# superxslam/SuperOdom

Measured on AMD Instinct MI355X. Metric: icp_registrations_per_sec, higher is better.
Workload: dtype f64

## Files before the change

### include/so_icp.h

```cpp
#ifndef SO_ICP_H
#define SO_ICP_H

#include <stddef.h>
#include <stdint.h>

#ifdef __cplusplus
extern "C" {
#endif

#define SO_ICP_ABI_VERSION 4

#define SO_ICP_MAP_W 21
#define SO_ICP_MAP_H 21
#define SO_ICP_MAP_D 11
#define SO_ICP_MAP_NUM 4851
#define SO_ICP_MAX_OUTER 16

#define SO_ICP_OK 0
#define SO_ICP_NOT_ENOUGH_MAP_FEATURES 1
#define SO_ICP_MAP_SEEDED 2
#define SO_ICP_STAGE_DECLINED 3
#define SO_ICP_E_INVALID (-1)
#define SO_ICP_E_HIP (-2)
#define SO_ICP_E_NOMEM (-3)
// ... 70 lines not shown
#define SO_ICP_FLAG_RETRIED 0x2u
#define SO_ICP_FLAG_HOST_MAP 0x4u
#define SO_ICP_FLAG_SORT_BINNING 0x8u
#define SO_ICP_FLAG_SHARDED 0x10u
#define SO_ICP_FLAG_STAGED_SCAN 0x20u
#define SO_ICP_FLAG_COPY_READBACK 0x40u
#define SO_ICP_FLAG_QUERY_SPLIT 0x80u
#define SO_ICP_FLAG_BINNED_AHEAD 0x100u
#define SO_ICP_FLAG_QUERY_WAVES 0x200u

#define SO_ICP_FLAG_CHAINED 0x400u
#define SO_ICP_FLAG_POSE_PRIOR 0x800u

typedef struct {
  double knn_ms_total;   int64_t knn_launches;   int64_t knn_queries;   int64_t knn_map_points;
  double eval_ms_total;  int64_t eval_launches;  int64_t eval_points;
  double prep_ms_total;  int64_t prep_launches;
  double host_ms_total;  int64_t registrations;
  int64_t knn_group_passes, knn_fallback_lanes, knn_candidates_scanned;
  double stage_wait_ms_total;  int64_t staged_direct, staged_copied, stage_declined;
  int64_t knn_packed_rows, knn_packed_rows_too_many_runs, knn_packed_rows_tile_full, knn_packed_kept;
  int64_t knn_pack_registrations, knn_pack_holds;
  int64_t seq_chained, seq_chain_breaks;
} so_icp_timing;

void so_icp_default_config(so_icp_config *cfg);
so_icp_ctx *so_icp_create(const so_icp_config *cfg);
void so_icp_destroy(so_icp_ctx *ctx);
const char *so_icp_last_error(const so_icp_ctx *ctx);
int so_icp_abi_version(void);
int so_icp_device_available(void);
int so_icp_device_count(void);

int so_icp_set_resolution(so_icp_ctx *ctx, float line_res, float plane_res);
int so_icp_set_max_surface_features(so_icp_ctx *ctx, int max_surface_features);
int so_icp_set_max_iterations(so_icp_ctx *ctx, int max_iterations);
int so_icp_set_cloud_intensity(so_icp_ctx *ctx, int offset_bytes);

int so_icp_map_set_origin(so_icp_ctx *ctx, const double t_w_cur[3], int origin_out[3]);
int so_icp_map_shift(so_icp_ctx *ctx, const double t_w_cur[3], int pos_in_map[3]);
int so_icp_map_add_surf(so_icp_ctx *ctx, const float *xyz, size_t n, size_t stride_bytes);
int so_icp_map_count_5x5(so_icp_ctx *ctx, const int pos[3], int *n_edge, int *n_surf);
int so_icp_map_export(so_icp_ctx *ctx, float *xyz, size_t cap_points, size_t *n_out, int only_5x5, const int pos[3]);
int so_icp_map_export_records(so_icp_ctx *ctx, void *out, size_t stride_bytes, size_t cap_points, size_t *n_out, int only_5x5, const int pos[3]);
int so_icp_map_size(so_icp_ctx *ctx, size_t *n_points, size_t *n_points_this_rank);
int so_icp_map_clear(so_icp_ctx *ctx);
// ... 302 lines not shown
```

### superodom_amd/binding.py

```python
import ctypes as C
import math
import os

import numpy as np

HERE = os.path.dirname(os.path.abspath(__file__))
LIB_PATH = os.path.join(HERE, "lib", "libsoicp.so")
N_REJECT, N_OBS, MAX_OUTER, UID_BYTES, PEER_HANDLE_BYTES = 7, 9, 16, 128, 80

OK, NOT_ENOUGH_MAP_FEATURES, MAP_SEEDED = 0, 1, 2
SHARD_MAP, SHARD_QUERIES = 0, 1


class Config(C.Structure):
    _fields_ = [("abi_version", C.c_int32), ("device_id", C.c_int32), ("rank", C.c_int32), ("world_size", C.c_int32),
                ("max_iterations", C.c_int32), ("lm_max_iterations", C.c_int32), ("max_surface_features", C.c_int32),
                ("k", C.c_int32), ("tukey_variant", C.c_int32), ("time_kernels", C.c_int32),
                ("line_res", C.c_float), ("plane_res", C.c_float), ("yaw_ratio", C.c_double),
                ("velocity_failure_threshold", C.c_double), ("shard_mode", C.c_int32), ("solve_workgroups", C.c_int32)]


class IterStats(C.Structure):
    _fields_ = [("translation_norm", C.c_double), ("rotation_norm", C.c_double), ("num_surf_from_scan", C.c_int32),
                ("num_corner_from_scan", C.c_int32), ("lm_iterations", C.c_int32), ("num_successful_steps", C.c_int32),
# ... 105 lines not shown
def untimed_layout(fields, point_step, row_step, n_scans, filter_point_size, min_range, is_bigendian=False):
    off = {}
    for name in ("x", "y", "z", "intensity"):
        for fname, foff, fdt, fcount in fields:
            if fname == name and fdt == FLOAT32 and (fcount == 1 or fcount == 0):
                off[name] = int(foff)
                break
    L = UntimedLayout()
    L.is_bigendian, L.point_step, L.row_step = int(bool(is_bigendian)), int(point_step), int(row_step)
    L.off_x, L.off_y, L.off_z, L.off_intensity = off.get("x", -1), off.get("y", -1), off.get("z", -1), off.get("intensity", -1)
    L.n_scans, L.filter_point_size, L.min_range = int(n_scans), int(filter_point_size), float(min_range)
    return L


class Timing(C.Structure):
    _fields_ = [("knn_ms_total", C.c_double), ("knn_launches", C.c_int64), ("knn_queries", C.c_int64), ("knn_map_points", C.c_int64),
                ("eval_ms_total", C.c_double), ("eval_launches", C.c_int64), ("eval_points", C.c_int64),
                ("prep_ms_total", C.c_double), ("prep_launches", C.c_int64),
                ("host_ms_total", C.c_double), ("registrations", C.c_int64),
                ("knn_group_passes", C.c_int64), ("knn_fallback_lanes", C.c_int64), ("knn_candidates_scanned", C.c_int64),
                ("stage_wait_ms_total", C.c_double), ("staged_direct", C.c_int64), ("staged_copied", C.c_int64), ("stage_declined", C.c_int64),
                ("knn_packed_rows", C.c_int64), ("knn_packed_rows_too_many_runs", C.c_int64), ("knn_packed_rows_tile_full", C.c_int64),
                ("knn_packed_kept", C.c_int64), ("knn_pack_registrations", C.c_int64), ("knn_pack_holds", C.c_int64),
                ("seq_chained", C.c_int64), ("seq_chain_breaks", C.c_int64)]


class Sums(C.Structure):
    _fields_ = [("cost", C.c_double), ("count", C.c_double), ("Jtr", C.c_double * 6), ("JtJ", C.c_double * 21), ("hist", C.c_double * 16)]


class LmState(C.Structure):
    _fields_ = [("opaque", C.c_double * 96)]


class LmScriptEntry(C.Structure):
    _fields_ = [("sums", Sums), ("new_solve", C.c_int32), ("reserved", C.c_int32)]


class LmScriptStep(C.Structure):
    _fields_ = [("more", C.c_int32), ("reserved", C.c_int32), ("pose", C.c_double * 7), ("hand", (C.c_uint32 * 4) * 8), ("state", LmState)]


class LmScriptResult(C.Structure):
    _fields_ = [("state", LmState), ("T", C.c_double * 7), ("eval_pose", C.c_double * 7), ("T_final", C.c_double * 7),
                ("JtJ", C.c_double * 36), ("Jtr", C.c_double * 6),
                ("lm_more", C.c_int32), ("outer_iter", C.c_int32), ("n_iterations", C.c_int32), ("reg_done", C.c_int32),
                ("done_count", C.c_uint32), ("reserved", C.c_uint32), ("iterations", IterStats * 16)]
# ... 984 lines not shown
```

### superodom_amd/csrc/ctx.h

```cpp
#pragma once
#include <hip/hip_runtime_api.h>
#include <rccl/rccl.h>

#include <atomic>
#include <chrono>
#include <condition_variable>
#include <cstdint>
#include <cstring>
#include <memory>
#include <mutex>
#include <string>
#include <thread>
#include <vector>

#include "../../include/so_icp.h"
#include "device_map.h"
#include "kernels.h"
#include "local_map.h"
#include "lm_solver.h"
#include "reg_plan.h"
#include "so_math.h"

namespace soicp::host {

// ... 252 lines not shown
  bool prebin = true;
  BinHashTable pbin;
  StageSlot* stage_in_use = nullptr;
  unsigned long long stage_seq = 0, stage_consumed_seq = 0;
  bool stage_quit = false, stage_started = false;
  std::atomic<int> stage_pending{0};
  std::atomic<bool> stage_parked{false};
  std::atomic<bool> stage_timed{false};
  std::thread stage_thread; std::mutex stage_mu; std::condition_variable stage_cv;
  struct HostRange { const char* p; size_t bytes; bool owned; };
  std::vector<HostRange> host_ranges;
  hipStream_t seq_stream = nullptr;
  StageSlot seq_slot[kStageSlots];
  BinHashTable sbin;
  int seq_depth = 2; uint32_t done_count_seen = 0;
  struct SeqNext { const void* next_scan = nullptr; size_t next_n = 0; double delta[7] = {0, 0, 0, 0, 0, 0, 1}; bool announced = false;
                   const void* scan = nullptr; size_t n = 0;
                   bool staged = false; int slot = 0; bool binned = false, needs_event = false; const float* d_scan = nullptr; } seq_next;
  bool seq_chain = true;
  bool query_waves = true;
  bool knn_pack = true;
  bool knn_list_fits = false;
  uint32_t packed_leftover_seen = 0;
  int knn_pack_hold = 0;
  static constexpr int kBatchRoundsTracked = 16;
  float batch_survivors[kBatchRoundsTracked] = {};
  bool batch_chain = true;
  hipStream_t copy_stream = nullptr;
  bool retried = false;
  unsigned long long peer_timeout_ticks = 100000000ull;
  bool scan_staged = false;
  bool query_split = false;
  DevBuf d_sub;

  ~so_icp_ctx();
};

#define HIP_TRY(ctx, expr)                                                                         \
  do {                                                                                             \
    hipError_t e__ = (expr);                                                                       \
    if (e__ != hipSuccess) {                                                                       \
      (ctx)->err = std::string(#expr) + ": " + hipGetErrorString(e__);                             \
      return SO_ICP_E_HIP;                                                                         \
    }                                                                                              \
  } while (0)

// ... 106 lines not shown
```

### superodom_amd/csrc/icp_context.cpp

```cpp
#include <hip/hip_runtime_api.h>

#include <algorithm>
#include <atomic>
#include <chrono>
#include <cmath>
#include <cstdlib>
#include <cstring>
#include <new>
#include <string>
#include <thread>
#include <vector>

#include "ctx.h"

static_assert(sizeof(so_icp_sums) == sizeof(LmSums), "so_icp_sums must mirror LmSums");
static_assert(sizeof(LmState) <= sizeof(so_icp_lm_state), "so_icp_lm_state too small");
static_assert(sizeof(LmSums) == 45 * sizeof(double), "LmSums is 45 doubles");

namespace soicp::host {

thread_local std::string g_create_error;

hipEvent_t next_event(so_icp_ctx* c) {
  if (c->ev_used == c->ev_pool.size()) {
// ... 149 lines not shown
  for (unsigned spin = 1;; ++spin) {
    if (*seq == want) break;
    if ((spin & 0x3FFu) != 0) continue;
    const auto now = std::chrono::steady_clock::now();
    if (now < next_check) continue;
    next_check = now + std::chrono::milliseconds(1);
    if (hipStreamQuery(s) != hipErrorNotReady) {
      (void)hipGetLastError();
      if (*seq == want) break;
      const hipError_t e = hipStreamSynchronize(s);
      if (e != hipSuccess) { c->err = std::string("hipStreamSynchronize(s): ") + hipGetErrorString(e); return Report::kHipError; }
      if (*seq == want) break;
      return Report::kDrained;
    }
  }
  std::atomic_thread_fence(std::memory_order_acquire);
  return Report::kReported;
}
void note_registration_done(so_icp_ctx* c, DevState* mirror, const MatchParams& mp, size_t n, bool sets_list_fits, bool sets_done_count) {
  const DevState& H = *(c->h_state = mirror);
  if (mp.pack_light) c->timing.knn_pack_registrations++;
  const uint32_t packed_left = H.packed_leftover >= c->packed_leftover_seen ? H.packed_leftover - c->packed_leftover_seen : H.packed_leftover;
  c->packed_leftover_seen = H.packed_leftover;
  if (mp.pack_light && (double)packed_left > 0.03 * (double)n * (double)std::max(H.n_iterations, 1)) { c->knn_pack_hold = 32; c->timing.knn_pack_holds++; }
  if (sets_list_fits) c->knn_list_fits = work_list_fits(H.bin_packed, (unsigned long long)kKnnBlocks * 4ull);
  if (sets_done_count) c->done_count_seen = H.done_count;
}

static void uncertainty_from_hist(const int32_t* H, double u[6]) {
  const double tt = (double)H[6] + H[7] + H[8];
  const double tr = (double)H[0] + H[1] + H[2] + H[3] + H[4] + H[5];
  if (tt == 0 || tr == 0) { for (int i = 0; i < 6; ++i) u[i] = 0; return; }
  u[0] = std::fmin(H[6] / tt * 3, 1.0); u[1] = std::fmin(H[7] / tt * 3, 1.0); u[2] = std::fmin(H[8] / tt * 3, 1.0);
  u[3] = std::fmin((H[0] + H[1]) / tr * 3, 1.0); u[4] = std::fmin((H[2] + H[3]) / tr * 3, 1.0); u[5] = std::fmin((H[4] + H[5]) / tr * 3, 1.0);
}

static void yaw_correction(double T[7], const double last[7], double yaw_ratio) {
  double tn, rn;
  relative_motion(last, T, tn, rn);
  const float translation_norm = (float)tn;
  const double x = T[3], y = T[4], z = T[5], w = T[6];
  const double d = x * x + y * y + z * z + w * w, s = 2.0 / d;
  const double xs = x * s, ys = y * s, zs = z * s, wx = w * xs, wy = w * ys, wz = w * zs;
  const double xx = x * xs, xy = x * ys, xz = x * zs, yy = y * ys, yz = y * zs, zz = z * zs;
  const double m00 = 1.0 - (yy + zz), m01 = xy - wz, m02 = xz + wy, m10 = xy + wz, m20 = xz - wy, m21 = yz + wx, m22 = 1.0 - (xx + yy);
  double roll, pitch, yaw;
// ... 936 lines not shown
```

### superodom_amd/csrc/kernels.h

```cpp
#pragma once
#include <hip/hip_runtime_api.h>

#include <cstddef>
#include <cstdint>

#include "lm_endgame.h"
#include "lm_solver.h"
#include "pose_prior.h"
#include "so_math.h"

#ifndef SO_ENDGAME_IMAGE
#define SO_ENDGAME_IMAGE 1
#endif
#ifndef SO_PUBLISH_FENCED
#define SO_PUBLISH_FENCED 0
#endif
#ifndef SO_PTOL_AT_PROPOSAL
#define SO_PTOL_AT_PROPOSAL 1
#endif

namespace soicp {

struct DevMapView {
  const float4* pts;
// ... 47 lines not shown
  unsigned long long timeout_ticks;
};
constexpr int kPeerMaxWorld = 8, kPeerChunks = 48;
constexpr size_t kPeerInboxBytes = (size_t)(2 * kPeerMaxWorld * kPeerChunks + kPeerMaxWorld) * 16;

struct CorrBuffers {
  double4* nd;
  double* coeff;
  uint8_t* status;
};

struct DevIterStats {
  double translation_norm, rotation_norm;
  int32_t num_surf, lm_iterations, num_successful, termination;
  double initial_cost, final_cost;
  int32_t reject_hist[7], obs_hist[9];
  double pose_after[7];
};
struct DevState {
  double pose_in[7];
  int32_t max_outer, lm_max, pad0, pad1;
  int32_t outer_iter, reg_done, lm_more, n_iterations;
  uint32_t packed_leftover;
  uint32_t pad2[3];
  unsigned long long bin_packed;
  double T[7];
  double eval_pose[7];
  LmState S;
  double JtJ[36], Jtr[6];
  DevIterStats iters[16];
  double T_final[7];
  double T_chain[7];
  uint32_t done_count, pad3;
  unsigned long long peer_seq;
  unsigned long long dbg[16];
  unsigned long long seq;
};
static_assert(sizeof(DevState) % 8 == 0, "DevState is copied in 8-byte words");

constexpr int kHistReplicas = 16;
constexpr int kHistStride = 32;
constexpr int kKnnBlocks = 1024;
#ifndef SO_SOLVE_BLOCKS
#define SO_SOLVE_BLOCKS 256
#endif
constexpr int kEvalBlocks = SO_SOLVE_BLOCKS;
constexpr int kFitBlocksMax = SO_SOLVE_BLOCKS;
// ... 86 lines not shown
```

### superodom_amd/csrc/kernels.hip

```cpp
#include <hip/hip_runtime.h>
#include <hip/hip_ext.h>

#include <cstddef>
#include <cstdlib>
#include <cstring>
#include <type_traits>

#ifdef SO_LM_STAMPS
#define SO_LM_STAMP(dbg, i) do { if (dbg) (dbg)[i] = wall_clock64(); } while (0)
#endif
#include "device_idioms.h"
#include "kernels.h"
#include "plane_factor.h"
#include "plane_fit.h"
#include "pose_prior.h"

namespace soicp {

#define SO_MATCH_SUCCESS 0
#define SO_MATCH_NOT_ENOUGH 1
#define SO_MATCH_TOO_FAR 2
#define SO_MATCH_BAD_PCA 3
#define SO_MATCH_INVALID 4
#define SO_MATCH_MSE 5
// ... 407 lines not shown
__device__ __forceinline__ float block_cover_distance(int bx0, int bx1, int by0, int by1, int bz0, int bz1, int nc, float cell,
                                                      float ux, float uy, float uz) {
  float cv = 1e15f;
  if (bx0 > 0) cv = fminf(cv, ux - (float)bx0 * cell);
  if (bx1 < nc - 1) cv = fminf(cv, (float)(bx1 + 1) * cell - ux);
  if (by0 > 0) cv = fminf(cv, uy - (float)by0 * cell);
  if (by1 < nc - 1) cv = fminf(cv, (float)(by1 + 1) * cell - uy);
  if (bz0 > 0) cv = fminf(cv, uz - (float)bz0 * cell);
  if (bz1 < nc - 1) cv = fminf(cv, (float)(bz1 + 1) * cell - uz);
  return fmaxf(cv - 1e-4f, 0.f);
}
__device__ __forceinline__ void survivors_to_canon(const Net8& net, const uint32_t* tile_canon, uint32_t n_valid, uint32_t tile_cap,
                                                   uint32_t (&canon)[8]) {
  const int32_t ks[8] = {net.a0, net.a1, net.a2, net.a3, net.a4, net.a5, net.a6, net.a7};
#pragma unroll
  for (int t = 0; t < 8; ++t) {
    const uint32_t jl = (uint32_t)ks[t] & kKeyIdxMask;
    canon[t] = (ks[t] == kKeyEmpty || jl >= n_valid) ? 0xFFFFFFFFu : tile_canon[jl < tile_cap ? jl : 0u];
  }
}
#ifndef SO_KNN_PACK
#define SO_KNN_PACK 1
#endif
constexpr uint32_t kPartTile = kTileCand / 4;

template <bool PROF, bool BATCH, int BEGIN = 0>
__global__ __launch_bounds__(256, 4) void knn_plane_kernel(const float4* __restrict__ binned ,
                                                        const uint32_t* __restrict__ chunk_start,
                                                        const DevState* __restrict__ st,
                                                        const float4* __restrict__ mpts,
                                                        const uint32_t* __restrict__ mcell_start, DevMapView map,
                                                        MatchParams mp, CorrBuffers corr, uint32_t* __restrict__ nbr5,
                                                        int32_t* __restrict__ hist, BatchView bv) {
  __shared__ int32_t lh[24];
  __shared__ __attribute__((aligned(16))) float tiles[4][4][kTileCand + 16];
  __shared__ uint32_t tcanon[4][kTileCand + 16];
  __shared__ uint32_t rowtab[4][2][72];
  unsigned long long t_entry = 0;
  if (PROF) t_entry = wall_clock64();
  if (SO_ENTRY_WARM) st = after_loaded(st, kernarg_lines<decltype(&knn_plane_kernel<PROF, BATCH, BEGIN>)>());
  if (BATCH) {
    const size_t h = bv.active[blockIdx.y];
    st += h; binned += h * bv.bs; chunk_start += h * bv.bs;
    corr.status += h * bv.bs; nbr5 += h * 5 * bv.bs; hist += h * (kHistReplicas * kHistStride);
  }
  uint32_t* const leftover_ctr = (BATCH && mp.packed_leftover)
      ? reinterpret_cast<uint32_t*>(reinterpret_cast<char*>(mp.packed_leftover) + (size_t)bv.active[blockIdx.y] * sizeof(DevState)) : mp.packed_leftover;
  constexpr bool begin = BEGIN != 0 && !BATCH;
// ... 54 lines not shown
  if (stamp) { ts[0] = wall_clock64(); if (!n_mine) t_item0 = ts[0]; }
  uint32_t j = 0;
  bool valid_q = false;
  bool split = false, split4 = false;
  const uint32_t part = (uint32_t)lane >> 4, lane16 = (uint32_t)lane & 15u;
  if constexpr (packed) {
    const uint32_t li = chunk * 4u + part;
    const uint32_t desc = li < n_light ? chunk_start[mp.chunk_cap - 1u - li] : 0u;
    const uint32_t start = desc & 0x03FFFFFFu, count = li < n_light ? (desc >> 26) + 1u : 0u;
    j = start + lane16;
    valid_q = (lane16 < count) && (j < n_kept);
  } else {
    const uint32_t entry = pack ? chunk - n_packed
                         : (chunk < n_light1 ? mp.chunk_cap - 1u - chunk
                            : (chunk < n_light1 + n_normal ? chunk - n_light1 : mp.chunk_cap - 1u - (chunk - n_normal)));
    const uint32_t desc = __builtin_amdgcn_readfirstlane(chunk_start[entry]);
    const uint32_t start = desc & 0x03FFFFFFu, count = (desc >> 26) + 1u;
    split = count <= 32u && !(abl & 1024);
    split4 = count <= 16u && split && !(abl & 2048);
    const int ql = split4 ? (lane & 15) : (split ? (lane & 31) : lane);
    j = start + (uint32_t)ql;
    valid_q = (ql < (int)count) && (j < n_kept);
  }
  const uint32_t hoff = split4 ? (uint32_t)(lane >> 4) << 2 : (split ? (uint32_t)(lane >> 5) << 2 : 0u);
  const uint32_t sstep = split4 ? 16u : 8u;
  double pw[3] = {0, 0, 0};
  float qx = 0, qy = 0, qz = 0;
  float ux = 0, uy = 0, uz = 0;
  int wcube0 = 0, wcube1 = 0, wcube2 = 0;
  CellRef c;
  c.slot = -1; c.cx = c.cy = c.cz = 0;
  uint32_t oi = 0;
  if (valid_q) {
    const float4 rec = binned[j];
    oi = __float_as_uint(rec.w);
    quat_rotate<double>(pose.q, (double)rec.x, (double)rec.y, (double)rec.z, pw[0], pw[1], pw[2]);
    pw[0] += pose.t[0]; pw[1] += pose.t[1]; pw[2] += pose.t[2];
    qx = (float)pw[0]; qy = (float)pw[1]; qz = (float)pw[2];
    int w[3] = {0, 0, 0};
    c = locate(map, qx, qy, qz, w);
    if (c.slot >= 0) {
      ux = (float)((double)qx - (w[0] * 50.0 - 25.0)); uy = (float)((double)qy - (w[1] * 50.0 - 25.0)); uz = (float)((double)qz - (w[2] * 50.0 - 25.0));
      wcube0 = w[0]; wcube1 = w[1]; wcube2 = w[2];
    }
  }
  const uint32_t ckey = (valid_q && c.slot >= 0) ? (((uint32_t)c.slot << 18) | ((uint32_t)c.cz << 12) | ((uint32_t)c.cy << 6) | (uint32_t)c.cx)
                                                 : 0xFFFFFFFFu;
  Top5 top;
  top.init();
  bool resolved = (ckey == 0xFFFFFFFFu);
  bool too_far_certain = false, need_exact = false;
  int n_groups = 0;
  uint32_t n_scanned = 0, n_left_stat = 0;
  if (stamp) { ts[1] = wall_clock64(); acc[0] += ts[1] - ts[0]; }
  auto certify = [qx, qy, qz, mpts, &mp](int pass, const uint32_t (&gs)[8], int32_t k6, int32_t k8, float cov2, Top5& top) -> int {
    unsigned long long e[5];
#pragma unroll
    for (int t = 0; t < 5; ++t) {
      e[t] = ~0ull;
      if (gs[t] != 0xFFFFFFFFu) {
        const float4 p = mpts[gs[t]];
        e[t] = ((unsigned long long)__float_as_uint(l2_d2(qx, qy, qz, p.x, p.y, p.z)) << 32) | gs[t];
      }
    }
    top.set5(e[0], e[1], e[2], e[3], e[4]);
    const double cov = (double)cov2 * (1.0 - 1e-6);
    double R2 = cov;
    if (k6 != kKeyEmpty) R2 = fmin(R2, (double)__uint_as_float((uint32_t)k6 & ~kKeyIdxMask) * (1.0 - 1e-6) - (double)kApproxAbsErr);
    bool have5 = top.b4 != ~0ull;
    double d5 = (double)__uint_as_float((uint32_t)(top.b4 >> 32));
    bool exact = have5 && d5 < R2;
    bool far = !exact && R2 > (double)mp.sq_max_dist_f;
    if (__ballot(!exact && !far && gs[5] != 0xFFFFFFFFu)) {
      if (!exact && !far) {
#pragma unroll
        for (int t = 5; t < 8; ++t) {
// ... 23 lines not shown
    const bool mine = pend && myslot == gslot;
    const float r_cover = ppass == 0 ? r_near : r_gate;
    const int lo_x = max(0, (int)floorf((ux - r_cover) * inv_cellf)), hi_x = min(nc - 1, (int)floorf((ux + r_cover) * inv_cellf));
    const int lo_y = max(0, (int)floorf((uy - r_cover) * inv_cellf)), hi_y = min(nc - 1, (int)floorf((uy + r_cover) * inv_cellf));
    const int lo_z = max(0, (int)floorf((uz - r_cover) * inv_cellf)), hi_z = min(nc - 1, (int)floorf((uz + r_cover) * inv_cellf));
    const int bx0 = row_min_i32(mine ? lo_x : 0x7FFFFFFF), bx1 = row_max_i32(mine ? hi_x : -1);
    const int by0 = row_min_i32(mine ? lo_y : 0x7FFFFFFF), by1 = row_max_i32(mine ? hi_y : -1);
    const int bz0 = row_min_i32(mine ? lo_z : 0x7FFFFFFF), bz1 = row_max_i32(mine ? hi_z : -1);
    const int nyr = by1 - by0 + 1, nrows = nyr * (bz1 - bz0 + 1);
    bool part_ok = gslot != 0x7FFFFFFF && nrows >= 1 && nrows <= 16;
    float cv = block_cover_distance(bx0, bx1, by0, by1, bz0, bz1, nc, cell, ux, uy, uz);
    if (ppass == 1) cv = 1e15f;
    const float cov2p = fminf(cv * cv, r_cover * r_cover);
    uint32_t vb = 0, vl = 0;
    if (part_ok && (int)lane16 < nrows) {
      const int zq = (int)(((float)lane16 + 0.5f) * __builtin_amdgcn_rcpf((float)nyr));
      const int z = bz0 + zq, y = by0 + ((int)lane16 - zq * nyr);
      const uint32_t* row = mcell_start + (size_t)gslot * map.ncell1 + ((size_t)z * nc + y) * nc;
      vb = row[bx0]; vl = row[bx1 + 1] - vb;
    }
    const uint32_t inc = row_inclusive_scan_u32(vl);
    const uint32_t total = (uint32_t)row_max_i32((int)inc);
    part_ok = part_ok && total <= 1024u;
    uint32_t* prowoff = rowoff + part * 17u;
    uint32_t* prowbeg = rowbeg + part * 16u;
    wave_lds_fence();
    prowoff[lane16] = ((int)lane16 < nrows) ? inc - vl : total; prowbeg[lane16] = vb;
    if (lane16 == 0) prowoff[16] = total;
    const int gz = (bz0 + bz1) >> 1, gy = (by0 + by1) >> 1, gx = (bx0 + bx1) >> 1;
    const int w0r = row_max_i32(mine ? wcube0 : -0x7FFFFFFF), w1r = row_max_i32(mine ? wcube1 : -0x7FFFFFFF), w2r = row_max_i32(mine ? wcube2 : -0x7FFFFFFF);
    const double rox = (w0r * 50.0 - 25.0) + ((double)gx + 0.5) * (double)cell;
    const double roy = (w1r * 50.0 - 25.0) + ((double)gy + 0.5) * (double)cell;
    const double roz = (w2r * 50.0 - 25.0) + ((double)gz + 0.5) * (double)cell;
    const float lqx = (float)((double)qx - rox), lqy = (float)((double)qy - roy), lqz = (float)((double)qz - roz);
    const float m2qx = -2.f * lqx, m2qy = -2.f * lqy, m2qz = -2.f * lqz;
    const float qq = __builtin_fmaf(lqz, lqz, __builtin_fmaf(lqy, lqy, lqx * lqx));
    const float pinf = __int_as_float(0x7F800000);
    const float bl0 = row_min_f32(mine ? lqx : pinf), bl1 = row_min_f32(mine ? lqy : pinf), bl2 = row_min_f32(mine ? lqz : pinf);
    const float bh0 = -row_min_f32(mine ? -lqx : pinf), bh1 = -row_min_f32(mine ? -lqy : pinf), bh2 = -row_min_f32(mine ? -lqz : pinf);
    const float dk = r_cover + 2e-4f, dk2 = dk * dk;
    const uint32_t tbase = part * kPartTile;
    const uint32_t tot_eff = part_ok ? total : 0u;
    const uint32_t tmax = max_over_rows(tot_eff);
    wave_lds_fence();
    if (PROF) n_scanned += tmax;
    uint32_t w = 0;
// ... 143 lines not shown
      if (lane == L) {
        top.b0 = m5[0]; top.b1 = m5[1]; top.b2 = m5[2]; top.b3 = m5[3]; top.b4 = m5[4];
        too_far_certain = false; resolved = true;
      }
  };
  if constexpr (packed) {
    unsigned long long left = __ballot(valid_q && c.slot >= 0 && !resolved);
    if (left) __builtin_amdgcn_s_setprio(3);
    if (left && lane == 0 && mp.packed_leftover) atomicAdd(leftover_ctr, (uint32_t)__popcll(left));
    if (PROF) n_left_stat = (uint32_t)__popcll(left);
    while (left) {
      const int L = __ffsll((long long)left) - 1;
      left &= left - 1ull;
      coop_exact_scan(L);
    }
  }
  if constexpr (!packed)
  for (int pass = first_pass; pass < 2; ++pass) {
  bool pending = !resolved && !need_exact;
  unsigned long long todo = __ballot(pending);
  if (abl & 2) todo = 0;
  if (!todo) continue;
  if (pass == 1 && first_pass == 0) __builtin_amdgcn_s_setprio(3);
  if (stamp && pass == 1) ++n_pass2;
  const float r_cover = pass == 0 ? r_near : r_gate;
  const int lo_x = max(0, (int)floorf((ux - r_cover) * inv_cellf)), hi_x = min(nc - 1, (int)floorf((ux + r_cover) * inv_cellf));
  const int lo_y = max(0, (int)floorf((uy - r_cover) * inv_cellf)), hi_y = min(nc - 1, (int)floorf((uy + r_cover) * inv_cellf));
  const int lo_z = max(0, (int)floorf((uz - r_cover) * inv_cellf)), hi_z = min(nc - 1, (int)floorf((uz + r_cover) * inv_cellf));
  uint32_t g0 = 0xFFFFFFFFu, g1 = g0, g2 = g0, g3 = g0, g4 = g0, g5 = g0, g6 = g0, g7 = g0;
  int32_t k6 = kKeyEmpty, k8 = kKeyEmpty;
  float cov2 = 0.f;
  bool scanned = false;
  while (todo) {
    const int leader = __ffsll((long long)todo) - 1;
    const uint32_t k = __builtin_amdgcn_readlane(ckey, leader);
    const int gslot = (int)(k >> 18);
    bool mine = pending && ((int)(ckey >> 18) == gslot);
    int bx0, bx1, by0, by1, bz0, bz1;
    uint32_t total = 0;
    uint32_t vb = 0, vl = 0;
    int nrows = 0, nyr = 0;
    const int lcx = (int)(k & 63u), lcy = (int)((k >> 6) & 63u), lcz = (int)((k >> 12) & 63u);
    for (int attempt = 0; attempt < 3; ++attempt) {
      if (attempt == 1)
        mine = mine && abs(c.cx - lcx) <= 1 && abs(c.cy - lcy) <= 1 && abs(c.cz - lcz) <= 1;
      if (attempt == 2) mine = mine && (ckey == k);
      bx0 = __builtin_amdgcn_readlane(lo_x, leader); bx1 = __builtin_amdgcn_readlane(hi_x, leader);
// ... 23 lines not shown
        if (lane == 0) rowoff[32] = total;
      }
      if (total <= kGroupMaxCand) break;
    }
    pending = pending && !mine;
    todo = __ballot(pending);
    ++n_groups;
    if (total > kGroupMaxCand) {
      need_exact = need_exact || mine;
      continue;
    }
    n_scanned += total;
    if (n_scanned > 256u) __builtin_amdgcn_s_setprio(3);
    else if (n_scanned > 128u) __builtin_amdgcn_s_setprio(2);
    if (stamp) { ts[2] = wall_clock64(); acc[1] += ts[2] - ts[1]; }
    const int gz = (bz0 + bz1) >> 1, gy = (by0 + by1) >> 1, gx = (bx0 + bx1) >> 1;
    const double ox = ((int)__builtin_amdgcn_readlane(wcube0, leader) * 50.0 - 25.0) + ((double)gx + 0.5) * (double)cell;
    const double oy = ((int)__builtin_amdgcn_readlane(wcube1, leader) * 50.0 - 25.0) + ((double)gy + 0.5) * (double)cell;
    const double oz = ((int)__builtin_amdgcn_readlane(wcube2, leader) * 50.0 - 25.0) + ((double)gz + 0.5) * (double)cell;
    const float lqx = (float)((double)qx - ox), lqy = (float)((double)qy - oy), lqz = (float)((double)qz - oz);
    const float m2qx = -2.f * lqx, m2qy = -2.f * lqy, m2qz = -2.f * lqz;
    const float qq = __builtin_fmaf(lqz, lqz, __builtin_fmaf(lqy, lqy, lqx * lqx));
    const uint32_t keep = ~kKeyIdxMask;
    const float2v pqx = {m2qx, m2qx}, pqy = {m2qy, m2qy}, pqz = {m2qz, m2qz}, pqq = {qq, qq};
    Net8 net;
    net.init();
    bool filt = SO_KNN_FILTER != 0;
    float bl0 = 0.f, bl1 = 0.f, bl2 = 0.f, bh0 = 0.f, bh1 = 0.f, bh2 = 0.f;
    if (filt) {
      const float pinf = __int_as_float(0x7F800000);
      bl0 = wave_min_f32(mine ? lqx : pinf); bl1 = wave_min_f32(mine ? lqy : pinf); bl2 = wave_min_f32(mine ? lqz : pinf);
      bh0 = -wave_min_f32(mine ? -lqx : pinf); bh1 = -wave_min_f32(mine ? -lqy : pinf); bh2 = -wave_min_f32(mine ? -lqz : pinf);
    }
    const float dk = r_cover + 2e-4f, dk2 = dk * dk;
    uint32_t total_eff = total;
    if (filt) {
      wave_lds_fence();
      uint32_t w = 0;
      for (uint32_t t0 = 0; t0 < total; t0 += 64) {
        const uint32_t t = t0 + (uint32_t)lane;
        bool kp = false;
        float lx = 0.f, ly = 0.f, lz = 0.f, lc = 0.f;
        uint32_t canon = 0xFFFFFFFFu;
        if (t < total) {
          int r = 0;
#pragma unroll
          for (int step = 16; step >= 1; step >>= 1) r = (r + step < 32 && rowoff[r + step] <= t) ? r + step : r;
          canon = rowbeg[r] + (t - rowoff[r]);
          const float4 p = mpts[canon];
          lx = (float)((double)p.x - ox); ly = (float)((double)p.y - oy); lz = (float)((double)p.z - oz);
          lc = __builtin_fmaf(lz, lz, __builtin_fmaf(ly, ly, lx * lx));
          const float ex = fmaxf(fmaxf(bl0 - lx, lx - bh0), 0.f), ey = fmaxf(fmaxf(bl1 - ly, ly - bh1), 0.f), ez = fmaxf(fmaxf(bl2 - lz, lz - bh2), 0.f);
          kp = __builtin_fmaf(ez, ez, __builtin_fmaf(ey, ey, ex * ex)) <= dk2;
        }
        const unsigned long long m = __ballot(kp);
// ... 13 lines not shown
    const uint32_t n_enum = filt ? total_eff : total;
    for (uint32_t base = 0; base < n_enum; base += kTileCand) {
      const uint32_t cnt = (n_enum - base < kTileCand) ? n_enum - base : kTileCand;
      wave_lds_fence();
      if (filt) {
      } else
      if (!(abl & 16))
      for (uint32_t t = lane; t < cnt + 16; t += 64) {
        float lx = 0.f, ly = 0.f, lz = 0.f, lc = 3.0e38f;
        uint32_t canon = 0xFFFFFFFFu;
        if (t < cnt) {
          const uint32_t e = base + t;
          int r = 0;
#pragma unroll
          for (int step = 16; step >= 1; step >>= 1) r = (r + step < 32 && rowoff[r + step] <= e) ? r + step : r;
          canon = rowbeg[r] + (e - rowoff[r]);
          const float4 p = mpts[canon];
          lx = (float)((double)p.x - ox); ly = (float)((double)p.y - oy); lz = (float)((double)p.z - oz);
          lc = __builtin_fmaf(lz, lz, __builtin_fmaf(ly, ly, lx * lx));
        }
        tx[t] = lx; ty[t] = ly; tz[t] = lz; tc[t] = lc; ti[t] = canon;
      }
      wave_lds_fence();
      if (!(abl & 8) && split) {
        for (uint32_t jl = 0; jl < cnt; jl += sstep) {
          const uint32_t a = jl + hoff;
          const float4 X = *reinterpret_cast<const float4*>(tx + a), Y = *reinterpret_cast<const float4*>(ty + a);
          const float4 Z = *reinterpret_cast<const float4*>(tz + a), C = *reinterpret_cast<const float4*>(tc + a);
          const float2v d01 = approx_d2_pair(pqx, pqy, pqz, pqq, float2v{X.x, X.y}, float2v{Y.x, Y.y}, float2v{Z.x, Z.y}, float2v{C.x, C.y});
          const float2v d23 = approx_d2_pair(pqx, pqy, pqz, pqq, float2v{X.z, X.w}, float2v{Y.z, Y.w}, float2v{Z.z, Z.w}, float2v{C.z, C.w});
          const uint32_t e = base + a;
          net.push(make_key_v(d01.x, e, keep));
          net.push(make_key_v(d01.y, e + 1, keep));
          net.push(make_key_v(d23.x, e + 2, keep));
          net.push(make_key_v(d23.y, e + 3, keep));
        }
      } else if (!(abl & 8)) {
        float4 X = *reinterpret_cast<const float4*>(tx), Y = *reinterpret_cast<const float4*>(ty);
        float4 Z = *reinterpret_cast<const float4*>(tz), C = *reinterpret_cast<const float4*>(tc);
        for (uint32_t jl = 0; jl < cnt; jl += 4) {
          const uint32_t nx = (jl + 4 < cnt) ? jl + 4 : jl;
          const float4 Xn = *reinterpret_cast<const float4*>(tx + nx), Yn = *reinterpret_cast<const float4*>(ty + nx);
          const float4 Zn = *reinterpret_cast<const float4*>(tz + nx), Cn = *reinterpret_cast<const float4*>(tc + nx);
          const float2v d01 = approx_d2_pair(pqx, pqy, pqz, pqq, float2v{X.x, X.y}, float2v{Y.x, Y.y}, float2v{Z.x, Z.y}, float2v{C.x, C.y});
          const float2v d23 = approx_d2_pair(pqx, pqy, pqz, pqq, float2v{X.z, X.w}, float2v{Y.z, Y.w}, float2v{Z.z, Z.w}, float2v{C.z, C.w});
          const uint32_t e = base + jl;
          net.push(make_key(d01.x, e, keep));
          net.push(make_key(d01.y, e + 1, keep));
          net.push(make_key(d23.x, e + 2, keep));
          net.push(make_key(d23.y, e + 3, keep));
          X = Xn; Y = Yn; Z = Zn; C = Cn;
        }
      }
    }
    if (split) {
      const int32_t o0 = __shfl_xor(net.a0, 32, 64), o1 = __shfl_xor(net.a1, 32, 64), o2 = __shfl_xor(net.a2, 32, 64), o3 = __shfl_xor(net.a3, 32, 64);
      const int32_t o4 = __shfl_xor(net.a4, 32, 64), o5 = __shfl_xor(net.a5, 32, 64), o6 = __shfl_xor(net.a6, 32, 64), o7 = __shfl_xor(net.a7, 32, 64);
      net.push(o0); net.push(o1); net.push(o2); net.push(o3); net.push(o4); net.push(o5); net.push(o6); net.push(o7);
      if (split4) {
        const int32_t p0 = __shfl_xor(net.a0, 16, 64), p1 = __shfl_xor(net.a1, 16, 64), p2 = __shfl_xor(net.a2, 16, 64), p3 = __shfl_xor(net.a3, 16, 64);
        const int32_t p4 = __shfl_xor(net.a4, 16, 64), p5 = __shfl_xor(net.a5, 16, 64), p6 = __shfl_xor(net.a6, 16, 64), p7 = __shfl_xor(net.a7, 16, 64);
        net.push(p0); net.push(p1); net.push(p2); net.push(p3); net.push(p4); net.push(p5); net.push(p6); net.push(p7);
      }
    }
    if (stamp) { ts[3] = wall_clock64(); acc[2] += ts[3] - ts[2]; }
    uint32_t gi[8];
    if (filt || total <= kTileCand) {
      survivors_to_canon(net, ti, total_eff, kTileCand, gi);
    } else {
      const int32_t ks[8] = {net.a0, net.a1, net.a2, net.a3, net.a4, net.a5, net.a6, net.a7};
#pragma unroll
      for (int t = 0; t < 8; ++t) {
        const uint32_t jl = (uint32_t)ks[t] & kKeyIdxMask;
        int r = 0;
#pragma unroll
        for (int step = 16; step >= 1; step >>= 1) r = (r + step < 32 && rowoff[r + step] <= jl) ? r + step : r;
        gi[t] = (ks[t] == kKeyEmpty || jl >= total) ? 0xFFFFFFFFu : rowbeg[r] + (jl - rowoff[r]);
      }
    }
    if (mine) {
      g0 = gi[0]; g1 = gi[1]; g2 = gi[2]; g3 = gi[3]; g4 = gi[4]; g5 = gi[5]; g6 = gi[6]; g7 = gi[7];
      k6 = net.a5; k8 = net.a7;
      scanned = true;
      if (pass == 1) {
        cov2 = 1e30f;
      } else {
        const float cv = block_cover_distance(bx0, bx1, by0, by1, bz0, bz1, nc, cell, ux, uy, uz);
        cov2 = cv * cv;
      }
      if (filt) cov2 = fminf(cov2, r_cover * r_cover);
    }
    if (stamp) { ts[1] = wall_clock64(); acc[3] += ts[1] - ts[3]; }
  }
  if (scanned && !need_exact && !(abl & 4)) {
    const uint32_t gs[8] = {g0, g1, g2, g3, g4, g5, g6, g7};
    const int v = certify(pass, gs, k6, k8, cov2, top);
    if (v == 1 || v == 2) resolved = true;
    if (v == 2) too_far_certain = true;
    if (v == 3) need_exact = true;
  } else if (scanned && (abl & 4)) {
    resolved = true;
  }
  }
  if (stamp) ts[2] = wall_clock64();
  __builtin_amdgcn_s_setprio(0);
// ... 10 lines not shown
  }
  if (valid_q && (!split || lane < (split4 ? 16 : 32))) {
    int status;
    if (c.slot < 0) {
      status = SO_MATCH_NOT_ENOUGH;
    } else {
      const float d2_4 = __uint_as_float((uint32_t)(top.b4 >> 32));
      if ((abl & 1) || too_far_certain || top.b4 == ~0ull || (double)d2_4 > (double)mp.sq_max_dist_f) {
        status = SO_MATCH_TOO_FAR;
      } else {
        status = SO_MATCH_PENDING;
        uint32_t* o = nbr5 + (size_t)5 * oi;
        __builtin_nontemporal_store((uint32_t)top.b0, o); __builtin_nontemporal_store((uint32_t)top.b1, o + 1);
        __builtin_nontemporal_store((uint32_t)top.b2, o + 2); __builtin_nontemporal_store((uint32_t)top.b3, o + 3);
        __builtin_nontemporal_store((uint32_t)top.b4, o + 4);
      }
    }
    __builtin_nontemporal_store((uint8_t)status, &corr.status[oi]);
  }
  if (stamp) {
    asm volatile("s_waitcnt vmcnt(0)" ::: "memory");
    ts[3] = wall_clock64(); acc[4] += ts[3] - ts[2]; ++n_mine;
    const unsigned long long nfb = packed ? n_left_stat : __popcll(__ballot(valid_q && c.slot >= 0 && (need_exact || !resolved)));
    if (ts[3] - ts[0] > t_maxchunk) { t_maxchunk = ts[3] - ts[0]; max_info = ((unsigned long long)n_scanned << 32) | (nfb << 16) | (unsigned long long)n_groups; }
    n_fb_total += nfb;
    n_cand_total += n_scanned; n_groups_total += n_groups; n_q_total += __popcll(__ballot(valid_q));
  }
  };
  for (uint32_t chunk = blockIdx.x * 4 + wv; chunk < n_chunks; chunk += gridDim.x * 4) {
    if (SO_KNN_PACK && chunk < n_packed) do_item(std::true_type{}, chunk); else do_item(std::false_type{}, chunk);
  }
  if (stamp && lane_k == 0) {
    unsigned long long* d = mp.kdbg + ((size_t)(begin ? 0 : (st->outer_iter & 1)) * gridDim.x * 4 + blockIdx.x * 4 + wv) * 16;
    d[0] = t_first; d[1] = wall_clock64();
    for (int i = 0; i < 5; ++i) d[2 + i] = acc[i];
    d[15] = clock64() - c_first;
    d[7] = n_mine; d[8] = t_maxchunk; d[9] = n_cand_total; d[10] = n_q_total; d[11] = n_groups_total; d[13] = max_info;
    d[12] = n_pass2 | ((t_item0 ? t_item0 - t_entry : 0ull) << 32);
    d[14] = n_fb_total | ((unsigned long long)(__builtin_amdgcn_s_getreg(63492) & 0xFFFFu) << 32) | ((unsigned long long)(__builtin_amdgcn_s_getreg(63508) & 0xFu) << 48);
  }
  if (PROF) {
    __syncthreads();
    if (threadIdx.x >= 16 && threadIdx.x < 24 && lh[threadIdx.x])
      atomicAdd(&hist[(blockIdx.x % kHistReplicas) * kHistStride + threadIdx.x], lh[threadIdx.x]);
  }
}

// ... 1555 lines not shown
```

Measured before the change: 8132.

## Repack sparse pass-2 KNN queries into 16-lane groups for 4-way candidate split

When a wave's second (gate) KNN pass has at most 16 owning queries, the query coordinates are compacted onto 16 lane slots and each candidate tile is split four ways across lane groups. The per-group top-8 networks are then merged with xor shuffles and the results shuffled back to their owning lanes. This targets poor lane utilisation on sparse fallback passes. It adds shuffle and merge overhead and extra profiling counters, plus a repacked-pass counter in the timing struct.

Result: no change. 8128 (-0.1%).

```diff
diff --git a/include/so_icp.h b/include/so_icp.h
--- a/include/so_icp.h
+++ b/include/so_icp.h
@@ -116,6 +116,7 @@
   int64_t knn_packed_rows, knn_packed_rows_too_many_runs, knn_packed_rows_tile_full, knn_packed_kept;
   int64_t knn_pack_registrations, knn_pack_holds;
   int64_t seq_chained, seq_chain_breaks;
+  int64_t knn_repacked_passes;
 } so_icp_timing;
 
 void so_icp_default_config(so_icp_config *cfg);
diff --git a/superodom_amd/binding.py b/superodom_amd/binding.py
--- a/superodom_amd/binding.py
+++ b/superodom_amd/binding.py
@@ -151,7 +151,8 @@
                 ("stage_wait_ms_total", C.c_double), ("staged_direct", C.c_int64), ("staged_copied", C.c_int64), ("stage_declined", C.c_int64),
                 ("knn_packed_rows", C.c_int64), ("knn_packed_rows_too_many_runs", C.c_int64), ("knn_packed_rows_tile_full", C.c_int64),
                 ("knn_packed_kept", C.c_int64), ("knn_pack_registrations", C.c_int64), ("knn_pack_holds", C.c_int64),
-                ("seq_chained", C.c_int64), ("seq_chain_breaks", C.c_int64)]
+                ("seq_chained", C.c_int64), ("seq_chain_breaks", C.c_int64),
+                ("knn_repacked_passes", C.c_int64)]
 
 
 class Sums(C.Structure):
diff --git a/superodom_amd/csrc/ctx.h b/superodom_amd/csrc/ctx.h
--- a/superodom_amd/csrc/ctx.h
+++ b/superodom_amd/csrc/ctx.h
@@ -298,6 +298,7 @@
   bool knn_pack = true;
   bool knn_list_fits = false;
   uint32_t packed_leftover_seen = 0;
+  uint32_t repacked_seen = 0;
   int knn_pack_hold = 0;
   static constexpr int kBatchRoundsTracked = 16;
   float batch_survivors[kBatchRoundsTracked] = {};
diff --git a/superodom_amd/csrc/icp_context.cpp b/superodom_amd/csrc/icp_context.cpp
--- a/superodom_amd/csrc/icp_context.cpp
+++ b/superodom_amd/csrc/icp_context.cpp
@@ -195,6 +195,8 @@
   if (mp.pack_light) c->timing.knn_pack_registrations++;
   const uint32_t packed_left = H.packed_leftover >= c->packed_leftover_seen ? H.packed_leftover - c->packed_leftover_seen : H.packed_leftover;
   c->packed_leftover_seen = H.packed_leftover;
+  c->timing.knn_repacked_passes += (int64_t)(uint32_t)(H.repacked_passes - c->repacked_seen);
+  c->repacked_seen = H.repacked_passes;
   if (mp.pack_light && (double)packed_left > 0.03 * (double)n * (double)std::max(H.n_iterations, 1)) { c->knn_pack_hold = 32; c->timing.knn_pack_holds++; }
   if (sets_list_fits) c->knn_list_fits = work_list_fits(H.bin_packed, (unsigned long long)kKnnBlocks * 4ull);
   if (sets_done_count) c->done_count_seen = H.done_count;
diff --git a/superodom_amd/csrc/kernels.h b/superodom_amd/csrc/kernels.h
--- a/superodom_amd/csrc/kernels.h
+++ b/superodom_amd/csrc/kernels.h
@@ -93,7 +93,8 @@
   int32_t max_outer, lm_max, pad0, pad1;
   int32_t outer_iter, reg_done, lm_more, n_iterations;
   uint32_t packed_leftover;
-  uint32_t pad2[3];
+  uint32_t repacked_passes;
+  uint32_t pad2[2];
   unsigned long long bin_packed;
   double T[7];
   double eval_pose[7];
diff --git a/superodom_amd/csrc/kernels.hip b/superodom_amd/csrc/kernels.hip
--- a/superodom_amd/csrc/kernels.hip
+++ b/superodom_amd/csrc/kernels.hip
@@ -453,8 +453,15 @@
 #ifndef SO_KNN_PACK
 #define SO_KNN_PACK 1
 #endif
+#ifndef SO_KNN_REPACK
+#define SO_KNN_REPACK 1
+#endif
 constexpr uint32_t kPartTile = kTileCand / 4;
 
+__device__ __forceinline__ unsigned long long stamp_item_info(bool packed, uint32_t queries, uint32_t cand, uint32_t fb, uint32_t groups, uint32_t detail) {
+  return (unsigned long long)min(groups, 255u) | ((unsigned long long)min(queries, 127u) << 8) | ((unsigned long long)(packed ? 1u : 0u) << 15) |
+         ((unsigned long long)min(fb, 0xFFFFu) << 16) | ((unsigned long long)min(cand, 0xFFFFFu) << 32) | ((unsigned long long)min(detail, 0xFFFu) << 52);
+}
 template <bool PROF, bool BATCH, int BEGIN = 0>
 __global__ __launch_bounds__(256, 4) void knn_plane_kernel(const float4* __restrict__ binned ,
                                                         const uint32_t* __restrict__ chunk_start,
@@ -555,8 +562,6 @@
     j = start + (uint32_t)ql;
     valid_q = (ql < (int)count) && (j < n_kept);
   }
-  const uint32_t hoff = split4 ? (uint32_t)(lane >> 4) << 2 : (split ? (uint32_t)(lane >> 5) << 2 : 0u);
-  const uint32_t sstep = split4 ? 16u : 8u;
   double pw[3] = {0, 0, 0};
   float qx = 0, qy = 0, qz = 0;
   float ux = 0, uy = 0, uz = 0;
@@ -584,7 +589,7 @@
   bool resolved = (ckey == 0xFFFFFFFFu);
   bool too_far_certain = false, need_exact = false;
   int n_groups = 0;
-  uint32_t n_scanned = 0, n_left_stat = 0;
+  uint32_t n_scanned = 0, n_left_stat = 0, stat_detail = 0, stat_near = 0, stat_pend_near = 255;
   if (stamp) { ts[1] = wall_clock64(); acc[0] += ts[1] - ts[0]; }
   auto certify = [qx, qy, qz, mpts, &mp](int pass, const uint32_t (&gs)[8], int32_t k6, int32_t k8, float cov2, Top5& top) -> int {
     unsigned long long e[5];
@@ -654,6 +659,8 @@
     const uint32_t inc = row_inclusive_scan_u32(vl);
     const uint32_t total = (uint32_t)row_max_i32((int)inc);
     part_ok = part_ok && total <= 1024u;
+    if (PROF && stamp && ppass == 0) { uint32_t m = gslot != 0x7FFFFFFF ? total : 0u; m = max(m, (uint32_t)__shfl_xor((int)m, 16, 64)); stat_detail = max(m, (uint32_t)__shfl_xor((int)m, 32, 64)); stat_near = gslot != 0x7FFFFFFF ? total : 0u; }
+    if (PROF && stamp && ppass == 1) { uint32_t m = pend ? min(stat_near, 254u) : 255u; for (int o = 1; o < 64; o <<= 1) m = min(m, (uint32_t)__shfl_xor((int)m, o, 64)); stat_pend_near = m; }
     uint32_t* prowoff = rowoff + part * 17u;
     uint32_t* prowbeg = rowbeg + part * 16u;
     wave_lds_fence();
@@ -843,7 +850,7 @@
   if (abl & 2) todo = 0;
   if (!todo) continue;
   if (pass == 1 && first_pass == 0) __builtin_amdgcn_s_setprio(3);
-  if (stamp && pass == 1) ++n_pass2;
+  if (stamp && pass == 1) { ++n_pass2; if constexpr (!packed) stat_detail = (uint32_t)__popcll(todo); }
   const float r_cover = pass == 0 ? r_near : r_gate;
   const int lo_x = max(0, (int)floorf((ux - r_cover) * inv_cellf)), hi_x = min(nc - 1, (int)floorf((ux + r_cover) * inv_cellf));
   const int lo_y = max(0, (int)floorf((uy - r_cover) * inv_cellf)), hi_y = min(nc - 1, (int)floorf((uy + r_cover) * inv_cellf));
@@ -913,7 +920,7 @@
     const float m2qx = -2.f * lqx, m2qy = -2.f * lqy, m2qz = -2.f * lqz;
     const float qq = __builtin_fmaf(lqz, lqz, __builtin_fmaf(lqy, lqy, lqx * lqx));
     const uint32_t keep = ~kKeyIdxMask;
-    const float2v pqx = {m2qx, m2qx}, pqy = {m2qy, m2qy}, pqz = {m2qz, m2qz}, pqq = {qq, qq};
+    float2v pqx = {m2qx, m2qx}, pqy = {m2qy, m2qy}, pqz = {m2qz, m2qz}, pqq = {qq, qq};
     Net8 net;
     net.init();
     bool filt = SO_KNN_FILTER != 0;
@@ -922,6 +929,17 @@
       const float pinf = __int_as_float(0x7F800000);
       bl0 = wave_min_f32(mine ? lqx : pinf); bl1 = wave_min_f32(mine ? lqy : pinf); bl2 = wave_min_f32(mine ? lqz : pinf);
       bh0 = -wave_min_f32(mine ? -lqx : pinf); bh1 = -wave_min_f32(mine ? -lqy : pinf); bh2 = -wave_min_f32(mine ? -lqz : pinf);
+    }
+    auto owners = [&]() -> unsigned long long { return __ballot(mine) & (split ? 0xFFFFFFFFull : ~0ull); };
+    auto repacked = [&]() -> bool { return SO_KNN_REPACK && pass == 1 && !split4 && __popcll(owners()) <= 16; };
+    if (repacked()) {
+      int src = lane;
+      unsigned long long m = owners();
+      for (uint32_t slot = 0; m; ++slot, m &= m - 1ull)
+        if (lane16 == slot) src = __ffsll((long long)m) - 1;
+      const float rx = __shfl(m2qx, src, 64), ry = __shfl(m2qy, src, 64), rz = __shfl(m2qz, src, 64), rq = __shfl(qq, src, 64);
+      pqx = float2v{rx, rx}; pqy = float2v{ry, ry}; pqz = float2v{rz, rz}; pqq = float2v{rq, rq};
+      if (lane == 0 && mp.packed_leftover) atomicAdd(leftover_ctr + 1, 1u);
     }
     const float dk = r_cover + 2e-4f, dk2 = dk * dk;
     uint32_t total_eff = total;
@@ -981,9 +999,11 @@
         tx[t] = lx; ty[t] = ly; tz[t] = lz; tc[t] = lc; ti[t] = canon;
       }
       wave_lds_fence();
-      if (!(abl & 8) && split) {
-        for (uint32_t jl = 0; jl < cnt; jl += sstep) {
-          const uint32_t a = jl + hoff;
+      if (!(abl & 8) && (split || repacked())) {
+        const bool four = split4 || repacked();
+        const uint32_t ghoff = four ? (uint32_t)(lane >> 4) << 2 : (uint32_t)(lane >> 5) << 2, gsstep = four ? 16u : 8u;
+        for (uint32_t jl = 0; jl < cnt; jl += gsstep) {
+          const uint32_t a = jl + ghoff;
           const float4 X = *reinterpret_cast<const float4*>(tx + a), Y = *reinterpret_cast<const float4*>(ty + a);
           const float4 Z = *reinterpret_cast<const float4*>(tz + a), C = *reinterpret_cast<const float4*>(tc + a);
           const float2v d01 = approx_d2_pair(pqx, pqy, pqz, pqq, float2v{X.x, X.y}, float2v{Y.x, Y.y}, float2v{Z.x, Z.y}, float2v{C.x, C.y});
@@ -1012,11 +1032,11 @@
         }
       }
     }
-    if (split) {
+    if (split || repacked()) {
       const int32_t o0 = __shfl_xor(net.a0, 32, 64), o1 = __shfl_xor(net.a1, 32, 64), o2 = __shfl_xor(net.a2, 32, 64), o3 = __shfl_xor(net.a3, 32, 64);
       const int32_t o4 = __shfl_xor(net.a4, 32, 64), o5 = __shfl_xor(net.a5, 32, 64), o6 = __shfl_xor(net.a6, 32, 64), o7 = __shfl_xor(net.a7, 32, 64);
       net.push(o0); net.push(o1); net.push(o2); net.push(o3); net.push(o4); net.push(o5); net.push(o6); net.push(o7);
-      if (split4) {
+      if (split4 || repacked()) {
         const int32_t p0 = __shfl_xor(net.a0, 16, 64), p1 = __shfl_xor(net.a1, 16, 64), p2 = __shfl_xor(net.a2, 16, 64), p3 = __shfl_xor(net.a3, 16, 64);
         const int32_t p4 = __shfl_xor(net.a4, 16, 64), p5 = __shfl_xor(net.a5, 16, 64), p6 = __shfl_xor(net.a6, 16, 64), p7 = __shfl_xor(net.a7, 16, 64);
         net.push(p0); net.push(p1); net.push(p2); net.push(p3); net.push(p4); net.push(p5); net.push(p6); net.push(p7);
@@ -1037,9 +1057,16 @@
         gi[t] = (ks[t] == kKeyEmpty || jl >= total) ? 0xFFFFFFFFu : rowbeg[r] + (jl - rowoff[r]);
       }
     }
+    int32_t nk6 = net.a5, nk8 = net.a7;
+    if (repacked()) {
+      const int slot = (int)__popcll(owners() & ((1ull << (lane & (split ? 31 : 63))) - 1ull));
+#pragma unroll
+      for (int t = 0; t < 8; ++t) gi[t] = (uint32_t)__shfl((int)gi[t], slot, 64);
+      nk6 = __shfl(nk6, slot, 64); nk8 = __shfl(nk8, slot, 64);
+    }
     if (mine) {
       g0 = gi[0]; g1 = gi[1]; g2 = gi[2]; g3 = gi[3]; g4 = gi[4]; g5 = gi[5]; g6 = gi[6]; g7 = gi[7];
-      k6 = net.a5; k8 = net.a7;
+      k6 = nk6; k8 = nk8;
       scanned = true;
       if (pass == 1) {
         cov2 = 1e30f;
@@ -1096,7 +1123,7 @@
     asm volatile("s_waitcnt vmcnt(0)" ::: "memory");
     ts[3] = wall_clock64(); acc[4] += ts[3] - ts[2]; ++n_mine;
     const unsigned long long nfb = packed ? n_left_stat : __popcll(__ballot(valid_q && c.slot >= 0 && (need_exact || !resolved)));
-    if (ts[3] - ts[0] > t_maxchunk) { t_maxchunk = ts[3] - ts[0]; max_info = ((unsigned long long)n_scanned << 32) | (nfb << 16) | (unsigned long long)n_groups; }
+    if (ts[3] - ts[0] > t_maxchunk) { t_maxchunk = ts[3] - ts[0]; max_info = stamp_item_info(packed, (uint32_t)__popcll(__ballot(valid_q)), n_scanned, packed ? (min((uint32_t)nfb, 255u) | (stat_pend_near << 8)) : (uint32_t)nfb, (uint32_t)n_groups, stat_detail); }
     n_fb_total += nfb;
     n_cand_total += n_scanned; n_groups_total += n_groups; n_q_total += __popcll(__ballot(valid_q));
   }
```
